# yukw777/EILEV

Measured on AMD Instinct MI355X. Metric: clips/sec (8-frame, 16 in-context) encode+generate, eilev-blip2-opt-2.7b, higher is better.
Workload: dtype bf16

## Files before the change

eilev_amd/csrc/common.h:

```cpp
#pragma once
#include <hip/hip_runtime.h>
#include <stdint.h>

#include <type_traits>

#include "../../include/eilev.h"

typedef __bf16 bf16;
typedef __attribute__((ext_vector_type(8))) __bf16 bf16x8;
typedef __attribute__((ext_vector_type(4))) __bf16 bf16x4;
typedef __attribute__((ext_vector_type(2))) __bf16 bf16x2;
typedef __attribute__((ext_vector_type(4))) float f32x4;
typedef __attribute__((ext_vector_type(16))) float f32x16;

#define EILEV_HIP_CHECK(expr)                          \
    do {                                               \
        hipError_t _e = (expr);                        \
        if (_e != hipSuccess) return (int)_e;          \
    } while (0)

static inline int eilev_num_cu() {
    static int n = 0;
    if (!n) {
        int dev = 0, cu = 0;
// ... 211 lines not shown
    DBG_GEMM_NB_BLOCKS_ONLY = 1 << 30,

    DBG_ATTN_NO_COMPUTE = 1 << 0,
    DBG_ATTN_NO_PREFETCH = 1 << 1,
    DBG_ATTN_NO_FRAME = 1 << 2,
    DBG_ATTN_FRAME3 = 1 << 4,
    DBG_ATTN_NO_FRAME3 = 1 << 5,
    DBG_ATTN_V2_4WAVES = 1 << 6,
    DBG_ATTN_FRAME_STAMPS = 1 << 8,
    DBG_ATTN_FRAME3_STAMPS = 1 << 9,
    DBG_ATTN_HEAD_MAJOR = 1 << 10,
    DBG_ATTN_FRAME3_NO_STORES = 1 << 11,
};
enum GemmForce : int { FORCE_NONE = 0, FORCE_PP4 = 9, FORCE_W6 = 12, FORCE_64x128 = 13, FORCE_128x128 = 14, FORCE_SPLIT_K = 15 };

struct GemmArgs {
    const bf16 *A;
    int64_t lda;
    const bf16 *W;
    int64_t ldw;
    const bf16 *Wp = nullptr;
    int a_frag = 0, c_frag = 0, ln_frag = 0;
    int hm_tok = 0, hm_heads = 0, hm_hd = 0;
    const bf16 *bias;
    const bf16 *resid;
    int64_t ldr;
    void *C;
    int64_t ldc;
    int M, N, K;
    int epi;
    int out_f32;
    float scale;
    int scale_cols;
    int patch_group;
    int dbg;
    float *scratch;
    size_t scratch_bytes;
    const float *wscale = nullptr;
    const uint8_t *W8 = nullptr;
    bf16 *w8_scratch = nullptr;
    const uint8_t *A8 = nullptr;
    const float *ascale = nullptr;
    const float *ln_rows = nullptr;
    const float *ln_csum = nullptr;
    float *stat_out = nullptr;
    int64_t stat_ld = 0;
// ... 3 lines not shown
    int k_slice = 0;
    unsigned long long *trace = nullptr;
    int trace_tiles = 0;
};

__host__ __device__ static inline int64_t frag32_index(int row, int col) { return (int64_t)(col >> 5) * 1024 + row * 32 + (col & 31); }

#ifdef EILEV_PROBES
extern int g_gemm_form;
#define GEMM_FORM(code) (g_gemm_form = (g_gemm_form & ~0xffff) | (code))
#define GEMM_FORM_BIT(bit) (g_gemm_form |= (bit))
extern int g_gemm_ks;
#define GEMM_FORM_KS(n) (g_gemm_ks = (n))
#else
#define GEMM_FORM(code) ((void)0)
#define GEMM_FORM_BIT(bit) ((void)0)
#define GEMM_FORM_KS(n) ((void)0)
#endif
enum : int { GEMM_FORM_ROW_CHUNKS = 1 << 16, GEMM_FORM_W8_EXPANDED = 1 << 17, GEMM_FORM_SPLIT_K = 1 << 18, GEMM_FORM_REDUCE_LN = 1 << 19,
             GEMM_FORM_STREAM_LAYOUT = 1 << 20 };

int launch_gemm(const GemmArgs &g, int prof_kind, hipStream_t s);
bool gemm_rows32_takes(const GemmArgs &g);
int launch_pp4_ext(const GemmArgs &g, int grid, hipStream_t s);
#ifdef EILEV_PROBES
#define EILEV_TRACE_M16 true
#else
#define EILEV_TRACE_M16 false
#endif
static inline bool pp4_all_lean(const GemmArgs &g) {
    const bool scale_ok = g.scale_cols == 0 || (g.scale_cols % 16 == 0 && g.epi == 0 && !g.resid && !g.ln_rows && !g.stat_out);
    return g.N % 128 == 0 && !g.out_f32 && g.patch_group == 0 && scale_ok && !g.wscale && !g.ascale && !g.dbg && (!g.trace || EILEV_TRACE_M16);
}
static inline bool hm_takes(const GemmArgs &g) {
    return g.hm_tok >= 128 && g.hm_heads > 0 && g.hm_hd > 64 && g.hm_hd % 8 == 0 && g.N == 3 * g.hm_heads * g.hm_hd && g.ln_rows && g.epi == 0 && !g.resid &&
           !g.stat_out && !g.scale_cols && pp4_all_lean(g) && g.N % 64 == 0 && g.M % g.hm_tok == 0 && (int64_t)g.M * g.N * 2 < 0xfffffff0ll;
}
bool gemv_rows_ok(int M, int N, int K);
int launch_gemv_rows(int pro, const bf16 *x, int64_t ldx, const bf16 *gamma, const bf16 *beta, float eps, const float *part, int heads, int hd,
                     int nsplit, const bf16 *W, const bf16 *bias, const bf16 *resid, int64_t ldr, void *out, int64_t ldo, int out_f32, int M, int N,
                     int K, int epi, float scale, int scale_cols, hipStream_t s);
bool gemv1_ok(int N, int K, int pro);
int launch_gemv1(int pro, const bf16 *x, const bf16 *gamma, const bf16 *beta, float eps, const bf16 *W, const bf16 *bias, const bf16 *resid, void *out,
                 int out_f32, int N, int K, int epi, float scale, int scale_cols, hipStream_t s, const float *part = nullptr, int heads = 0, int hd = 0,
                 int nsplit = 0);
bool gemvm_ok(int M, int N, int K, int pro);
// ... 111 lines not shown
```

eilev_amd/csrc/gemm.hip:

```cpp
#include "gemm_common.h"
#include "gemm_tiled.h"
#include "gemm_pp4.h"
#include "gemm_w6.h"
#include "gemm_skinny.h"

int g_eilev_grid_cus = 0;
#ifdef EILEV_PROBES
int g_gemm_debug = 0;
extern "C" int eilev_debug_gemm_flags(int f) { g_gemm_debug = f; return 0; }
extern "C" int eilev_debug_grid_cus(int n) { g_eilev_grid_cus = n; return 0; }
int g_gemm_form = 0;
int g_gemm_ks = 0;
#endif
#ifdef EILEV_PROBES
unsigned long long *g_gemm_trace = nullptr;
int g_gemm_trace_tiles = 0;
extern "C" int eilev_debug_gemm_trace(void *buf, int tiles) { g_gemm_trace = (unsigned long long *)buf; g_gemm_trace_tiles = tiles; return 0; }
#endif

namespace {

#ifndef EILEV_A3_MIN_K
#define EILEV_A3_MIN_K 5120
#endif
// ... 44 lines not shown
    if ((g.K % 128) || g.lda != g.K || g.ldw != g.K || ((uintptr_t)g.A8 & 15) || ((uintptr_t)g.W8 & 15) || g.patch_group != 0 ||
        (int64_t)g.M * g.K >= kOffsetLimit || (int64_t)g.N * g.K >= kOffsetLimit)
        return EILEV_E_UNSUPPORTED;
    if (!g.out_f32 && ((g.ldc & 7) || (g.N & 3) || ((uintptr_t)g.C & 15) || (g.resid && ((g.ldr & 7) || ((uintptr_t)g.resid & 15))))) return EILEV_E_UNSUPPORTED;
    return profiled(launch_pp4, g, prof_kind, s);
}

bool w8_streams(const GemmArgs &g) { return g.M <= 32 && g.K % 256 == 0 && g.patch_group == 0; }
int w8_check(const GemmArgs &g) {
    if (!g.A || !g.C || !g.wscale || g.N <= 0 || g.K <= 0 || g.ldw != g.K || ((uintptr_t)g.W8 & 15) || (g.K & 15)) return EILEV_E_BADARG;
    if (!w8_streams(g) && !g.w8_scratch) return EILEV_E_WORKSPACE;
    return EILEV_OK;
}
int w8_expand(const GemmArgs &g, hipStream_t s) {
    const int64_t n16 = (int64_t)g.N * g.K / 16;
    hipLaunchKernelGGL(w8_expand_kernel, dim3((unsigned)ceil_div64(n16, 256)), dim3(256), 0, s, g.W8, g.w8_scratch, n16);
    EILEV_LAUNCH_CHECK();
    return EILEV_OK;
}

bool ln_fold(const GemmArgs &g) { return g.ln_rows != nullptr || g.stat_out != nullptr; }
bool skinny_dma_ok(const GemmArgs &g) { return g.K % 256 == 0 && (!(g.dbg & DBG_GEMM_SKINNY_NO_DMA) || g.W8); }
bool skinny_takes(const GemmArgs &g) { return (g.M <= 16 || (g.M <= 32 && skinny_dma_ok(g))) && g.patch_group == 0 && !ln_fold(g); }

int check_args(const GemmArgs &g) {
    if (!g.A || !g.W || !g.C || g.N <= 0 || g.K <= 0) return EILEV_E_BADARG;
    if ((g.K & 7) || (g.lda & 7) || (g.ldw & 7) || ((uintptr_t)g.A & 15) || ((uintptr_t)g.W & 15)) return EILEV_E_UNSUPPORTED;
    if (g.hm_tok && (!hm_takes(g) || !fits_offset(g.M, g.lda))) return EILEV_E_UNSUPPORTED;
    if (ln_fold(g) && (g.W8 || g.wscale || g.out_f32 || g.patch_group || g.scale_cols || g.K % BK || !fits_offset(g.N, g.ldw))) return EILEV_E_UNSUPPORTED;
    const bool skinny = skinny_takes(g);
    if ((g.a_frag || g.c_frag || g.ln_frag) && !skinny) return EILEV_E_UNSUPPORTED;
    if (!skinny && !g.out_f32 && ((g.ldc & 7) || (g.N & 3) || ((uintptr_t)g.C & 15) || (g.resid && ((g.ldr & 7) || ((uintptr_t)g.resid & 15))) ||
                                   (g.bias && ((uintptr_t)g.bias & 7))))
        return EILEV_E_UNSUPPORTED;
    return EILEV_OK;
}


int skinny_nbsel(const GemmArgs &g, int nb, int ks) {
    int nbsel = (g.dbg >> DBG_GEMM_NB_SHIFT) & 7;
    if (nbsel == 0 && g.M > 16) {
        const int wgs = (g.dbg & DBG_GEMM_NB_BLOCKS_ONLY) ? nb : nb * ks;
        nbsel = wgs >= 8 * 240 ? 8 : (wgs >= 4 * 240 ? 4 : (wgs >= 2 * 240 ? 2 : 1));
    }
    if (nbsel == 7) nbsel = 8;
    if (nbsel != 2 && nbsel != 4 && nbsel != 8) nbsel = 1;
    if (nbsel == 8 && g.M <= 16) nbsel = 4;
    return g.W8 ? 1 : nbsel;
}

template <int MB, int NB>
int launch_skinny_nb(const SkinnyArgs &a, int nb, hipStream_t s) {
    const size_t sm = 4 * 2 * 8192 + (size_t)2 * 4 * MB * 64 * 4 * 4;
// ... 118 lines not shown
    return g.N % 256 == 0 ? 1.06 * fill(tiles256) < fill(tm256 * ceil_div64(g.N, 128)) : tiles256 < 1024;
}

bool split_k_takes(const GemmArgs &g) {
    return g.out_f32 && !g.bias && !g.resid && g.epi == 0 && !g.wscale && g.scale_cols == 0 && g.patch_group == 0 && g.K % BK == 0 && g.K >= 8192 &&
           ceil_div64(g.M, 128) * ceil_div64(g.N, 128) <= 128 && fits_offset(g.M, g.lda) && fits_offset(g.N, g.ldw);
}
int launch_split_k(const GemmArgs &g, hipStream_t s) {
    const int tiles = (int)(ceil_div64(g.M, 128) * ceil_div64(g.N, 128)), nk = g.K / BK;
    int slices = 512 / tiles;
    slices = slices < 2 ? 2 : (slices > 16 ? 16 : slices);
    if (slices > nk / 8) slices = nk / 8 > 1 ? nk / 8 : 1;
    GemmArgs gs = g;
    gs.k_slice = (nk + slices - 1) / slices;
    slices = (nk + gs.k_slice - 1) / gs.k_slice;
    if (g.ldc == g.N) EILEV_HIP_CHECK(hipMemsetAsync(g.C, 0, (size_t)g.M * g.N * sizeof(float), s));
    else EILEV_HIP_CHECK(hipMemset2DAsync(g.C, (size_t)g.ldc * sizeof(float), 0, (size_t)g.N * sizeof(float), (size_t)g.M, s));
    GEMM_FORM(3000 + slices);
    return eilev_launch<gemm_glds_kernel<128, 128, 2, 2, 0, 2, 2, 0>>(dim3(tiles, slices), dim3(256), 2 * (128 + 128) * 128, s, gs);
}

bool t64x128_takes(const GemmArgs &g) { return ceil_div64(g.M, 128) * ceil_div64(g.N, 128) < 96 && g.M > 64; }

int launch_wide(const GemmArgs &g, hipStream_t s) {
    const int force = (g.dbg >> DBG_GEMM_FORCE_SHIFT) & 15;
    const bool no_dma = g.dbg & DBG_GEMM_NO_DMA;
    int cfg = tile_cfg(g);
    bool promoted = false;
    if (cfg == CFG_256x128_1S && g.K % BK == 0 && !(g.dbg & DBG_GEMM_NO_WIDE)) cfg = CFG_256x256, promoted = true;
    if (cfg == CFG_256x128 && w6_ok(g) && force == FORCE_NONE && !(g.dbg & (DBG_GEMM_NO_WIDE | DBG_GEMM_NO_W6 | DBG_GEMM_NO_DMA))) cfg = CFG_256x256, promoted = true;
    if (force == FORCE_PP4) cfg = CFG_256x256;
    if (force == FORCE_64x128 || force == FORCE_128x128 || force == FORCE_SPLIT_K) cfg = CFG_128x128;
    else if (force >= CFG_256x256 && force <= CFG_128x128) cfg = force;

    if (w6_ok(g) && (force == FORCE_W6 || (force == FORCE_NONE && cfg == CFG_256x256 && w6_pick(g) && !(g.dbg & (DBG_GEMM_NO_W6 | DBG_GEMM_NO_DMA)))))
        return launch_w6(g, s);
    switch (cfg) {
        case CFG_256x256:
            if (!(promoted && (g.dbg & DBG_GEMM_WIDE_TILED)) && (force == FORCE_NONE || force == FORCE_PP4) && !no_dma && g.K % BK == 0 && fits_offset(g.N, g.ldw))
                return launch_pp4(g, s);
            return launch_tiled<256, 256, 2, 4, 2, 2>(g, s);
        case CFG_256x128_1S: return launch_tiled<256, 128, 4, 2, 1, 4, 1>(g, s);
        case CFG_256x128: return launch_tiled<256, 128, 4, 2, 2, 2>(g, s);
        default:
            if (split_k_takes(g) && (force == FORCE_NONE || force == FORCE_SPLIT_K) && !no_dma) return launch_split_k(g, s);
            if ((force == FORCE_64x128 || (force == FORCE_NONE && t64x128_takes(g))) && g.M > 64 && !no_dma) return launch_tiled<64, 128, 1, 2, 2, 3>(g, s);
            return launch_tiled<128, 128, 2, 2, 2, 2>(g, s);
    }
}

}


static int launch_gemm_core(const GemmArgs &g_in, int prof_kind, hipStream_t s, bool *ln_done);

bool gemm_rows32_takes(const GemmArgs &g) {
    if (!g.A || !g.W || !g.C || g.W8 || g.wscale || g.M <= 16 || g.M > 32 || g.K % 256 || g.patch_group || g.ln_rows || g.stat_out) return false;
    if ((g.lda & 7) || (g.ldw & 7) || ((uintptr_t)g.A & 15) || ((uintptr_t)g.W & 15) || (g.dbg & DBG_GEMM_NO_ROWS32)) return false;
    SkinnyArgs a;
    a.g = g;
    a.mr = 32;
    int ks = 1, ksteps = 0, grid_x = 0;
    return rows32_plan(g, (g.N + 15) / 16, skinny_n_cu(), a, ks, ksteps, grid_x);
}

extern "C" int eilev_stream_layout_pack(const void *w, int64_t n, int64_t k, void *out, void *stream) {
    if (!w || !out || w == out || n < 1 || k < 1) return EILEV_E_BADARG;
    if (n > 0x7fffffff || k > 0x7fffffff || n * k > 0x7fffffff0ll) return EILEV_E_UNSUPPORTED;
    int ks = 0, ksteps = 0, grid_x = 0;
    if (!rows32_shape((int)n, (int)k, skinny_n_cu(), ks, ksteps, grid_x)) return EILEV_E_UNSUPPORTED;
    const int64_t chunks = n * (k >> 3);
    hipLaunchKernelGGL(stream_pack_kernel, dim3((unsigned)((chunks + 255) / 256)), dim3(256), 0, (hipStream_t)stream, (const bf16 *)w, (bf16 *)out, (int)n, (int)k, grid_x);
    EILEV_LAUNCH_CHECK();
    return EILEV_OK;
}

int launch_gemm(const GemmArgs &g, int prof_kind, hipStream_t s) {
    bool ln_done = false;
    if (g.ln_out && g.M > 0 && (g.out_f32 || g.patch_group || (g.N & 7) || g.N > 4096 || (g.ldc & 7))) return EILEV_E_UNSUPPORTED;
    const int rc = launch_gemm_core(g, prof_kind, s, &ln_done);
    if (rc != EILEV_OK || !g.ln_out || ln_done || g.M <= 0) return rc;
    if (g.out_f32 || g.patch_group) return EILEV_E_UNSUPPORTED;
    if (!g.ln_beta) return launch_rmsnorm(reinterpret_cast<const bf16 *>(g.C), g.ldc, g.ln_gamma, g.ln_out, g.N, g.M, g.N, g.ln_eps, s);
    return launch_layernorm(reinterpret_cast<const bf16 *>(g.C), g.ldc, g.ln_gamma, g.ln_beta, g.ln_out, g.N, g.M, g.N, g.ln_eps, s);
}

static int launch_gemm_core(const GemmArgs &g_in, int prof_kind, hipStream_t s, bool *ln_done) {
    GemmArgs g = with_probes(g_in);
    if (g.M <= 0) return EILEV_OK;
    if (g.A8) return launch_a8w8(g, prof_kind, s);
    if (g.W8) {
        const int rc = w8_check(g);
        if (rc != EILEV_OK) return rc;
        if (!w8_streams(g)) {
            const int rc_x = w8_expand(g, s);
            if (rc_x != EILEV_OK) return rc_x;
            GEMM_FORM_BIT(GEMM_FORM_W8_EXPANDED);
            GemmArgs e = g_in;
            e.W = g.w8_scratch;
            e.W8 = nullptr;
            return launch_gemm_core(e, prof_kind, s, ln_done);
        }
        g.W = reinterpret_cast<const bf16 *>(g.W8);
    }
    const int rc = check_args(g);
    if (rc != EILEV_OK) return rc;
    if (skinny_takes(g)) return launch_skinny(g, s, ln_done);
    if (const int64_t rows = chunk_rows(g)) return launch_row_chunks(g_in, rows, prof_kind, s);
    return profiled(ln_fold(g) ? launch_pp4 : launch_wide, g, prof_kind, s);
}

#ifdef EILEV_PROBES
struct EilevDebugGemmArgs {
    const void *A; int64_t lda;
    const void *W; int64_t ldw;
    const void *bias, *resid; int64_t ldr;
    void *C; int64_t ldc;
    int32_t M, N, K, epi, out_f32;
    float scale;
    int32_t scale_cols, patch_group, hm_tok, hm_heads, hm_hd, pad0;
    const float *wscale;
    const void *W8;
    void *w8_scratch;
    const void *A8;
    const float *ascale, *ln_rows, *ln_csum;
    float *stat_out; int64_t stat_ld;
    const void *ln_gamma, *ln_beta;
    void *ln_out;
    float ln_eps;
    int32_t pad1;
// ... 42 lines not shown
```

eilev_amd/csrc/gemm_pp4.h:

```cpp
#pragma once
#include "gemm_common.h"

namespace {

#ifndef EILEV_PP4_DEEP
#define EILEV_PP4_DEEP 1
#endif
template <int EPI, bool F8 = false, int LN = 0, int M16K = 0, bool A3 = false>
__global__ __launch_bounds__(512, 2) void gemm_pp4_kernel(const GemmArgs g) {
    constexpr bool M16 = M16K != 0, HT16 = M16K == 2;
    constexpr bool TALL = HT16 && !A3;
    constexpr int TALL_BM = 384;
    constexpr int HT_WM = TALL ? TALL_BM / 4 : 64, HT_TM16 = HT_WM / 16;
    static_assert(!M16 || !F8, "16 x 16 form: bf16 instances");
    constexpr int BM = 256, BN = 256, NWM = 2, NWN = 4, NW = 8;
    constexpr int WM = BM / NWM, WN = BN / NWN, TM = WM / 32, TN = WN / 32;
    constexpr int STEP = (BM + BN) * 128;
    constexpr int PC = 8;
    static_assert(!A3 || M16, "A3: lean epilogues only");
    constexpr int STG0 = A3 ? 2 * BM * 128 : 2 * STEP;

    extern __shared__ __attribute__((aligned(16))) char smem[];
    auto a_slot = [&](int st) { return smem + (A3 ? (st % 3) * (BM * 128) : (st & 1) * STEP); };
    auto w_slot = [&](int st) { return smem + (A3 ? 3 * (BM * 128) + (st & 1) * (BN * 128) : (st & 1) * STEP + BM * 128); };
// ... 254 lines not shown
            if (hm) {
                const int TOK = g.hm_tok, HD = g.hm_hd, NH = g.hm_heads, D3 = g.N / 3;
                const int n0 = cn0 + coff;
                const int plane = __builtin_amdgcn_readfirstlane(n0 / D3), rr = n0 - plane * D3;
                int2 ent;
                if (rr < NH * 64) {
                    ent.x = (plane * NH + (rr >> 6)) * TOK * HD + schunk * 8;
                    ent.y = 64;
                } else {
                    const int cph = (HD - 64) >> 3, jb = ((rr - NH * 64) >> 3) + schunk, hh = jb / cph;
                    ent.x = (plane * NH + hh) * TOK * HD + TOK * 64 + (jb - hh * cph) * 8;
                    ent.y = HD - 64;
                }
                const int fw = __builtin_amdgcn_readfirstlane(r0 / TOK);
                const int m0 = r0 + srow, f0 = m0 / TOK;
                hm_t = m0 - f0 * TOK;
                hm_str2 = __builtin_amdgcn_readfirstlane(ent.y * 2);
                hm_off = (unsigned)(((f0 - fw) * TOK * g.N + ent.x + hm_t * ent.y) * 2);
                hm_off_w = hm_off + (unsigned)(TOK * g.N * 2) - (unsigned)(TOK * hm_str2);
                const int64_t left = ((int64_t)g.M / TOK - fw) * TOK * g.N * 2;
                rch = uniform_rsrc(reinterpret_cast<bf16 *>(g.C) + (int64_t)fw * TOK * g.N, (int)(unsigned)(left < 0xfffffff0ll ? left : 0xfffffff0ll));
            }
        }
        u32x4_t rv[4];
        auto res_load = [&](int u) {
#pragma unroll
            for (int it = 0; it < 4; ++it) rv[it] = __builtin_amdgcn_raw_buffer_load_b128(rr, rs_voff, (u * 32 + it * 8) * (int)(g.ldr * 2), 0);
        };
        if constexpr (RES) res_load(0);
        bf16x4 biasr[M16 ? 1 : TN][4];
        bf16x4 biasr16[M16 ? TN16 : 1];
        if constexpr (M16) {
#pragma unroll
            for (int j = 0; j < TN16; ++j) {
                if (g.bias) biasr16[j] = *reinterpret_cast<const bf16x4 *>(g.bias + cn0 + coff + j * 16 + g4 * 4);
                else biasr16[j] = (bf16x4){(bf16)0.f, (bf16)0.f, (bf16)0.f, (bf16)0.f};
            }
        } else {
#pragma unroll
        for (int j = 0; j < TN; ++j)
#pragma unroll
            for (int q = 0; q < 4; ++q) {
                if (g.bias) biasr[j][q] = *reinterpret_cast<const bf16x4 *>(g.bias + cn0 + wn * WN + j * 32 + q * 8 + hi * 4);
                else biasr[j][q] = (bf16x4){(bf16)0.f, (bf16)0.f, (bf16)0.f, (bf16)0.f};
            }
        }
// ... 116 lines not shown
                    if (g4 == 0) __builtin_amdgcn_raw_buffer_store_b64(__builtin_bit_cast(u32x2_t, t), rst, (U * 32 + ib * 16 + l15) * 8, 0, 0);
                }
            } else if constexpr (LNP) {
                typedef __attribute__((ext_vector_type(2))) unsigned u32x2_t;
                const f32x2_t t = (f32x2_t){st1 + __shfl_xor(st1, 32), st2 + __shfl_xor(st2, 32)};
                if (hi == 0) __builtin_amdgcn_raw_buffer_store_b64(__builtin_bit_cast(u32x2_t, t), rst, (U * 32 + l31) * 8, 0, 0);
            }
            __builtin_amdgcn_sched_barrier(0);
            bf16x8 erb[2];
#pragma unroll
            for (int h2 = 0; h2 < 2; ++h2) {
#pragma unroll
                for (int b = 0; b < 2; ++b) {
                    const int row = (h2 * 2 + b) * 8 + srow;
                    erb[b] = *reinterpret_cast<const bf16x8 *>(stg + row * 128 + ((schunk ^ (row & 7)) << 4));
                }
                if (hm) {
                    if constexpr (HMI) {
#pragma unroll
                        for (int b = 0; b < 2; ++b) {
                            const int RO = U * 32 + (h2 * 2 + b) * 8;
                            const unsigned vo = hm_t + RO >= g.hm_tok ? hm_off_w : hm_off;
                            __builtin_amdgcn_raw_buffer_store_b128(__builtin_bit_cast(u32x4_t, erb[b]), rch, vo, RO * hm_str2, EILEV_HM_AUX);
                        }
                    }
                } else {
#pragma unroll
                for (int b = 0; b < 2; ++b)
                    __builtin_amdgcn_raw_buffer_store_b128(__builtin_bit_cast(u32x4_t, erb[b]), rc, st_voff, (U * 32 + (h2 * 2 + b) * 8) * (int)(g.ldc * 2), EILEV_ST_AUX);
                }
            }
            asm volatile("s_nop 1" ::: "memory");
            __builtin_amdgcn_sched_barrier(0);
        });
    };
#define PP_WAIT_LGKM0() __builtin_amdgcn_s_waitcnt(0xC07F)
#define PP_WAIT_LGKM0_VM0() __builtin_amdgcn_s_waitcnt(0x0070)
#define PP_WAIT_VM0() __builtin_amdgcn_s_waitcnt(0x0F70)
#define PP_BARRIER()                       \
    do {                                   \
        __builtin_amdgcn_sched_barrier(0); \
        __builtin_amdgcn_s_barrier();      \
        __builtin_amdgcn_sched_barrier(0); \
    } while (0)

    int t = blockIdx.x, m0, n0;
// ... 256 lines not shown
```

eilev_amd/csrc/opt.hip:

```cpp
#include "stages.h"

namespace {
inline int64_t opt_ws_rows(int64_t M) { return (M > 16 && M < 32) ? 32 : M; }

}

OptBufs carve_opt(const EilevDims *d, int64_t M, void *ws) {
    Carver cv{(char *)ws};
    OptBufs b;
    M = opt_ws_rows(M);
    b.h = cv.take<bf16>((size_t)M * d->t_hidden);
    b.x = cv.take<bf16>((size_t)M * d->t_hidden);
    b.att = cv.take<bf16>((size_t)M * d->t_hidden);
    b.qkv = cv.take<bf16>((size_t)M * 3 * d->t_hidden);
    b.ffn = cv.take<bf16>((size_t)M * d->t_ffn);
    b.pid = cv.take<int32_t>((size_t)M);
    b.scratch = cv.take<float>(kSkinnyScratch / sizeof(float));
    b.a8 = cv.take<uint8_t>((size_t)M * (d->t_ffn > d->t_hidden ? d->t_ffn : d->t_hidden));
    b.a8_scale = cv.take<float>((size_t)M);
    b.used = cv.used;
    return b;
}

extern "C" size_t eilev_opt_workspace_bytes(const EilevDims *d, int64_t batch, int64_t seq_len) {
// ... 9 lines not shown
    if (!w8 || !sc) return EILEV_E_BADARG;
    if (w->w8_act_fp8 && g.M > 32 && g.K % 128 == 0 && (int64_t)g.M * g.K < 0x7fff0000ll && (int64_t)g.N * g.K < 0x7fff0000ll) {
        RC(launch_quant_rows_e4m3(g.A, g.lda, b.a8, b.a8_scale, g.M, g.K, s));
        g.A8 = b.a8;
        g.ascale = b.a8_scale;
        g.lda = g.K;
        g.W8 = w8;
        g.wscale = sc;
        g.ldw = g.K;
        return EILEV_OK;
    }
    if (g.M > 32 || g.K % 256 != 0) {
        if (!w->w8_expand || w->w8_expand_bytes < (size_t)g.N * g.K * sizeof(bf16)) return EILEV_E_WORKSPACE;
        g.w8_scratch = (bf16 *)w->w8_expand;
    }
    g.W8 = w8;
    g.wscale = sc;
    g.ldw = g.K;
    return EILEV_OK;
}

}

int opt_qkv(const EilevDims *d, const EilevOptWeights *w, int l, const OptBufs &b, int64_t M, hipStream_t s, int a_frag) {
    const EilevOptLayer *L = &w->layers[l];
    const int D = d->t_hidden;
    const float scaling = 1.0f / sqrtf((float)(D / d->t_heads));
    const void *ws[3] = {L->q_w, L->k_w, L->v_w}, *bs[3] = {L->q_b, L->k_b, L->v_b};
    const bool bias_fused = packed(bs, 3, D);
    if (w->layers_w8) {
        if (!bias_fused && (L->q_b || L->k_b || L->v_b)) return EILEV_E_UNSUPPORTED;
        GemmArgs g = sk_gemm(b.scratch, b.x, D, nullptr, D, L->q_b, nullptr, 0, b.qkv, 3 * D, M, 3 * D, D, 0);
        g.scale = scaling; g.scale_cols = D;
        RC(use_w8(g, w, w->layers_w8[l].qkv_w8, w->layers_w8[l].qkv_scale, b, s));
        return launch_gemm(g, 5, s);
    }
    const bool fused = packed(ws, 3, (size_t)D * D) && bias_fused;
    for (int i = 0; i < (fused ? 1 : 3); ++i) {
        GemmArgs g = sk_gemm(b.scratch, b.x, D, ws[i], D, bs[i], nullptr, 0, b.qkv + i * D, 3 * D, M, fused ? 3 * D : D, D, 0);
        if (i == 0) { g.scale = scaling; g.scale_cols = D; }
        if (fused && w->layers_stream && M > 16 && M <= 32) g.Wp = (const bf16 *)w->layers_stream[l].qkv_s;
        g.a_frag = a_frag;
        RC(launch_gemm(g, 5, s));
    }
    return EILEV_OK;
}

int opt_tail(const EilevDims *d, const EilevOptWeights *w, int l, const OptBufs &b, int64_t M, hipStream_t s, const void *next_ln_w,
             const void *next_ln_b, int frag, bool dry) {
    const EilevOptLayer *L = &w->layers[l];
    const EilevOptLayerW8 *Q = w->layers_w8 ? &w->layers_w8[l] : nullptr;
    const int D = d->t_hidden, Ft = d->t_ffn;
    const EilevOptLayerStream *S = (w->layers_stream && !Q && M > 16 && M <= 32) ? &w->layers_stream[l] : nullptr;
    GemmArgs g = sk_gemm(b.scratch, b.att, D, L->o_w, D, L->o_b, b.h, D, b.h, D, M, D, D, 0);
    g.ln_gamma = (const bf16 *)L->ln2_w; g.ln_beta = (const bf16 *)L->ln2_b; g.ln_out = b.x; g.ln_eps = d->t_eps;
    if (S) g.Wp = (const bf16 *)S->o_s;
    g.a_frag = g.ln_frag = frag;
    if (dry && !gemm_rows32_takes(g)) return EILEV_E_UNSUPPORTED;
    if (Q) RC(use_w8(g, w, Q->o_w8, Q->o_scale, b, s));
    if (!dry) RC(launch_gemm(g, 5, s));
    g = sk_gemm(b.scratch, b.x, D, L->fc1_w, D, L->fc1_b, nullptr, 0, b.ffn, Ft, M, Ft, D, 2);
    if (S) g.Wp = (const bf16 *)S->fc1_s;
    g.a_frag = g.c_frag = frag;
    if (dry && !gemm_rows32_takes(g)) return EILEV_E_UNSUPPORTED;
    if (Q) RC(use_w8(g, w, Q->fc1_w8, Q->fc1_scale, b, s));
    if (!dry) RC(launch_gemm(g, 5, s));
    g = sk_gemm(b.scratch, b.ffn, Ft, L->fc2_w, Ft, L->fc2_b, b.h, D, b.h, D, M, D, Ft, 0);
    if (S) g.Wp = (const bf16 *)S->fc2_s;
    if (next_ln_w) {
        g.ln_gamma = (const bf16 *)next_ln_w; g.ln_beta = (const bf16 *)next_ln_b; g.ln_out = b.x; g.ln_eps = d->t_eps;
    }
    g.a_frag = frag;
    g.ln_frag = next_ln_w ? frag : 0;
    if (dry) return gemm_rows32_takes(g) ? EILEV_OK : EILEV_E_UNSUPPORTED;
    if (Q) RC(use_w8(g, w, Q->fc2_w8, Q->fc2_scale, b, s));
    return launch_gemm(g, 5, s);
}

namespace {
int g_decode_frag = 1;
}
int g_decode_rows = 1;
#ifdef EILEV_PROBES
extern "C" int eilev_debug_decode_rows(int on) { g_decode_rows = on; return 0; }
extern "C" int eilev_debug_decode_frag(int on) { g_decode_frag = on; return 0; }
#endif
namespace {

bool opt_qkv_packed(const EilevDims *d, const EilevOptWeights *w) {
    const int D = d->t_hidden;
    for (int l = 0; l < d->t_layers; ++l) {
        const EilevOptLayer *L = &w->layers[l];
        const void *ws[3] = {L->q_w, L->k_w, L->v_w}, *bs[3] = {L->q_b, L->k_b, L->v_b};
        if (!packed(ws, 3, (size_t)D * D) || !L->q_b || !packed(bs, 3, D)) return false;
    }
    return true;
}
bool opt_rows_usable(const EilevDims *d, const EilevOptWeights *w, int64_t M) {
    if (!g_decode_rows || w->layers_w8 || M > 2) return false;
    const int D = d->t_hidden;
    return gemv_rows_ok((int)M, D, D) && gemv_rows_ok((int)M, D, d->t_ffn) && (D / d->t_heads) % 8 == 0 && opt_qkv_packed(d, w);
}
bool opt_rows1_usable(const EilevDims *d, const EilevOptWeights *w, int64_t M, int64_t cap) {
    if (M != 1 || g_decode_rows == 3 || !opt_rows_usable(d, w, M)) return false;
    const int D = d->t_hidden;
    return gemv1_ok(3 * D, D, 1) && gemv1_ok(D, D, 0) && gemv1_ok(d->t_ffn, D, 1) && gemv1_ok(D, d->t_ffn, 0) && gemv1_ok(d->vocab, D, 1) &&
           attn_decode1_ok(1, (int)cap, D / d->t_heads);
}
// ... 75 lines not shown
            int nsplit = 0;
            RC(opt_rows_qkv(d, w, l, b, M, s));
            RC(launch_attn_decode(al, s, &nsplit));
            RC(opt_rows_tail(d, w, l, b, M, al.part, nsplit, s));
        }
        return opt_rows_head(d, w, b, M, logits, s);
    }
    const int D = d->t_hidden;
    for (int l = 0; l < d->t_layers; ++l) {
        const EilevOptLayer *L = &w->layers[l];
        DecodeAttnArgs al = at_block(a, l, kv_layer, gen_layer);
        al.out_frag = frag;
        if (l == 0) RC(launch_layernorm(b.h, D, (const bf16 *)L->ln1_w, (const bf16 *)L->ln1_b, b.x, D, M, D, d->t_eps, s));
        RC(opt_qkv(d, w, l, b, M, s, l > 0 ? frag : 0));
        RC(launch_attn_decode(al, s));
        const bool last = l + 1 == d->t_layers;
        RC(opt_tail(d, w, l, b, M, s, last ? w->final_ln_w : w->layers[l + 1].ln1_w, last ? w->final_ln_b : w->layers[l + 1].ln1_b, frag));
    }
    GemmArgs g = opt_lm_head(d, w, b, M, logits);
    g.a_frag = frag;
    return launch_gemm(g, 5, s);
}

int opt_blocks(const EilevDims *d, const EilevOptWeights *w, const OptBufs &b, const void *inputs_embeds, const int32_t *attn_mask, int64_t batch,
               int64_t rows, int64_t past_len, bool from_cache, void *kv_cache, int64_t kv_capacity, void *hidden, hipStream_t s) {
    const int D = d->t_hidden, H = d->t_heads, hd = D / H;
    const int64_t M = batch * rows, total = past_len + rows;
    RC(launch_pos_embed((const bf16 *)inputs_embeds, (const bf16 *)w->embed_positions, attn_mask, b.pid, b.h, (int)batch, (int)total, D,
                        s, (int)past_len));
    const KvCache kv(batch, D, kv_capacity);
    const size_t hs_bytes = (size_t)M * D * sizeof(bf16);
    for (int l = 0; l < d->t_layers; ++l) {
        const EilevOptLayer *L = &w->layers[l];
        bf16 *kc = kv.k((bf16 *)kv_cache, l), *vc = kv.v((bf16 *)kv_cache, l);
        if (hidden) RC(copy_hidden(hidden, l, b.h, hs_bytes, s));
        RC(launch_layernorm(b.h, D, (const bf16 *)L->ln1_w, (const bf16 *)L->ln1_b, b.x, D, M, D, d->t_eps, s));
        RC(opt_qkv(d, w, l, b, M, s));
        RC(launch_kv_write(b.qkv, kc, vc, (int)batch, (int)rows, H, hd, (int)kv_capacity, (int)total, nullptr, s, (int)past_len));
        AttnArgs a = from_cache ? attn_cache(b.qkv, 3 * D, kc, vc, kv_capacity, b.att, batch, H, rows, total, hd, 1.0f)
                                : attn_rows(b.qkv, 3 * D, b.qkv + D, 3 * D, b.qkv + 2 * D, 3 * D, b.att, batch, H, rows, total, hd, 1.0f);
        a.causal = 1; a.key_mask = attn_mask; a.mask_ld = total;
        RC(launch_attention(a, s));
        RC(opt_tail(d, w, l, b, M, s));
    }
    RC(launch_layernorm(b.h, D, (const bf16 *)w->final_ln_w, (const bf16 *)w->final_ln_b, b.x, D, M, D, d->t_eps, s));
    if (hidden) RC(copy_hidden(hidden, d->t_layers, b.x, hs_bytes, s));
    return EILEV_OK;
}

int opt_prefill_impl(const EilevDims *d, const EilevOptWeights *w, const void *inputs_embeds, const int32_t *attn_mask, int64_t batch,
                     int64_t seq_len, void *kv_cache, int64_t kv_capacity, float *logits_last, float *logits_all, void *hidden,
                     void *workspace, size_t workspace_bytes, void *stream) {
    if (!d || !w || !inputs_embeds || !attn_mask || !kv_cache || !workspace || batch <= 0 || seq_len <= 0) return EILEV_E_BADARG;
    if (seq_len > kv_capacity || seq_len > d->max_pos) return EILEV_E_BADARG;
    if (!dims_ok_opt(d)) return EILEV_E_UNSUPPORTED;
    if (workspace_bytes < eilev_opt_workspace_bytes(d, batch, seq_len)) return EILEV_E_WORKSPACE;
    hipStream_t s = (hipStream_t)stream;
    const int D = d->t_hidden;
    const int64_t M = batch * seq_len;
    const OptBufs b = carve_opt(d, M, workspace);
    RC(opt_blocks(d, w, b, inputs_embeds, attn_mask, batch, seq_len, 0, false, kv_cache, kv_capacity, hidden, s));
    if (logits_all) {
        GemmArgs g = mk_gemm(b.x, D, w->embed_tokens, D, nullptr, nullptr, 0, logits_all, d->vocab, M, d->vocab, D, 0);
        g.out_f32 = 1;
        RC(launch_gemm(g, 5, s));
    }
    if (logits_last) {
        GemmArgs g = sk_gemm(b.scratch, b.x + (seq_len - 1) * (int64_t)D, seq_len * (int64_t)D, w->embed_tokens, D, nullptr, nullptr, 0,
                             logits_last, d->vocab, batch, d->vocab, D, 0);
        g.out_f32 = 1;
        RC(launch_gemm(g, 5, s));
    }
    return EILEV_OK;
}
}

extern "C" int eilev_opt_prefill(const EilevDims *d, const EilevOptWeights *w, const void *inputs_embeds,
                                 const int32_t *attn_mask, int64_t batch, int64_t seq_len, void *kv_cache, int64_t kv_capacity,
                                 float *logits_last, float *logits_all, void *workspace, size_t workspace_bytes, void *stream) {
    return opt_prefill_impl(d, w, inputs_embeds, attn_mask, batch, seq_len, kv_cache, kv_capacity, logits_last, logits_all, nullptr, workspace,
                            workspace_bytes, stream);
}
extern "C" int eilev_opt_prefill_debug(const EilevDims *d, const EilevOptWeights *w, const void *inputs_embeds,
                                       const int32_t *attn_mask, int64_t batch, int64_t seq_len, void *kv_cache, int64_t kv_capacity,
                                       float *logits_last, float *logits_all, void *hidden_states, void *workspace, size_t workspace_bytes,
                                       void *stream) {
    if (!hidden_states) return EILEV_E_BADARG;
    return opt_prefill_impl(d, w, inputs_embeds, attn_mask, batch, seq_len, kv_cache, kv_capacity, logits_last, logits_all, hidden_states,
                            workspace, workspace_bytes, stream);
}

extern "C" int eilev_opt_extend(const EilevDims *d, const EilevOptWeights *w, const void *inputs_embeds, const int32_t *attn_mask,
                                int64_t batch, int64_t new_len, int64_t past_len, void *kv_cache, int64_t kv_capacity,
                                float *logits_all, void *workspace, size_t workspace_bytes, void *stream) {
    if (!d || !w || !inputs_embeds || !attn_mask || !kv_cache || !logits_all || !workspace || batch <= 0 || new_len <= 0 || past_len < 0)
        return EILEV_E_BADARG;
    const int64_t total = past_len + new_len;
    if (total > kv_capacity || total > d->max_pos) return EILEV_E_BADARG;
    if (!dims_ok_opt(d)) return EILEV_E_UNSUPPORTED;
    if (workspace_bytes < eilev_opt_workspace_bytes(d, batch, total)) return EILEV_E_WORKSPACE;
    hipStream_t s = (hipStream_t)stream;
    const int D = d->t_hidden;
    const int64_t M = batch * new_len;
    const OptBufs b = carve_opt(d, batch * total, workspace);
    RC(opt_blocks(d, w, b, inputs_embeds, attn_mask, batch, new_len, past_len, true, kv_cache, kv_capacity, nullptr, s));
    GemmArgs g = sk_gemm(b.scratch, b.x, D, w->embed_tokens, D, nullptr, nullptr, 0, logits_all, d->vocab, M, d->vocab, D, 0);
    g.out_f32 = 1;
    return launch_gemm(g, 5, s);
}

extern "C" int eilev_greedy_select(const float *logits, int64_t batch, int64_t vocab, int32_t *state, uint8_t *finished,
                                   int64_t eos_id, int64_t pad_id, int64_t *tokens, int64_t *out_tokens, int64_t max_new,
                                   void *stream) {
    if (!logits || !state || !finished || !tokens || !out_tokens || batch <= 0) return EILEV_E_BADARG;
    return launch_select(logits, (int)batch, (int)vocab, state, finished, eos_id, pad_id, tokens, out_tokens, max_new,
                         (hipStream_t)stream);
}

extern "C" int eilev_topk_logprob(const float *logits, const float *row_score, int64_t rows, int64_t vocab, int64_t keep, float *out_val,
                                  int32_t *out_idx, void *stream) {
    if (!logits || !out_val || !out_idx || rows < 0 || vocab <= 0 || keep <= 0 || keep > vocab) return EILEV_E_BADARG;
    if (rows == 0) return EILEV_OK;
    return launch_topk_logprob(logits, row_score, (int)rows, (int)vocab, (int)keep, out_val, out_idx, (hipStream_t)stream);
}

extern "C" size_t eilev_beam_scratch_bytes(int64_t batch, int64_t beams, int64_t keep, int64_t max_new) {
    return sizeof(int64_t) * (size_t)batch * (size_t)(keep + 2 * beams) * (size_t)max_new;
}
// ... 125 lines not shown
```

eilev_amd/csrc/stages.h:

```cpp
#pragma once
#include "common.h"

#define RC(expr)                 \
    do {                         \
        int _rc = (expr);        \
        if (_rc != 0) return _rc; \
    } while (0)

struct Carver {
    char *base;
    size_t used = 0;
    template <typename T>
    T *take(size_t n) {
        T *q = base ? reinterpret_cast<T *>(base + used) : nullptr;
        used += align_up(n * sizeof(T), 256);
        return q;
    }
};

static inline GemmArgs mk_gemm(const bf16 *A, int64_t lda, const void *W, int64_t ldw, const void *bias, const bf16 *resid, int64_t ldr,
                               void *C, int64_t ldc, int64_t M, int N, int K, int epi) {
    GemmArgs g;
    g.A = A; g.lda = lda; g.W = (const bf16 *)W; g.ldw = ldw; g.bias = (const bf16 *)bias; g.resid = resid; g.ldr = ldr;
    g.C = C; g.ldc = ldc; g.M = (int)M; g.N = N; g.K = K; g.epi = epi; g.out_f32 = 0; g.scale = 1.0f; g.scale_cols = 0;
// ... 57 lines not shown
}

struct T5BeamArgs {
    int64_t beams;
    const void *kv_start;
    void *kv_gen;
    int64_t gen_capacity;
    const int32_t *ancestors;
};
int t5_decode_step_beam(const EilevT5Dims *d, const EilevT5Weights *w, const int64_t *tokens, int32_t *state, const int32_t *enc_mask,
                        int64_t rows, const T5BeamArgs &beam, const void *cross_kv, int64_t enc_len, float *logits, void *workspace,
                        size_t workspace_bytes, void *stream);
size_t t5_decode_step_beam_workspace_bytes(const EilevT5Dims *d, int64_t rows, int64_t enc_len, int64_t gen_capacity);

struct OptBufs {
    bf16 *h, *x, *att, *qkv, *ffn;
    int32_t *pid;
    float *scratch;
    uint8_t *a8;
    float *a8_scale;
    size_t used;
};
OptBufs carve_opt(const EilevDims *d, int64_t M, void *ws);
int opt_qkv(const EilevDims *d, const EilevOptWeights *w, int l, const OptBufs &b, int64_t M, hipStream_t s, int a_frag = 0);
int opt_tail(const EilevDims *d, const EilevOptWeights *w, int l, const OptBufs &b, int64_t M, hipStream_t s, const void *next_ln_w = nullptr,
             const void *next_ln_b = nullptr, int frag = 0, bool dry = false);

int opt_decode_step_beam(const EilevDims *d, const EilevOptWeights *w, const int64_t *tokens, int32_t *state, const int32_t *attn_mask,
                         const int32_t *n_valid, int64_t rows, int64_t beams, int64_t seq_len, const void *kv_prompt, void *kv_gen, int64_t gen_capacity,
                         const int32_t *ancestors, float *logits, void *workspace, size_t workspace_bytes, void *stream, int shared_prompt);
size_t opt_decode_step_beam_shared_bytes(const EilevDims *d, int64_t rows, int64_t seq_len, int64_t gen_capacity);

extern int g_decode_rows;
```

Baseline: 231.5.

## Write prefill K/V directly from QKV GEMM and compute only last rows in final layer

The fused QKV GEMM epilogue in the pp4 kernel can now store K and V columns straight into the KV cache layout, which removes the separate kv_write kernel during prompt prefill. Attention then reads K/V from the cache. In the last OPT layer, the output projection, FFN and final layernorm run only on each sequence's last row, because only last-token logits are needed. Tile routing keeps the full-M shape so the smaller GEMMs still pick the same kernels. This adds epilogue complexity and a routing override, and relies on the last-rows path being used only when the full hidden states and all-position logits are not requested.

```diff
diff --git a/eilev_amd/csrc/common.h b/eilev_amd/csrc/common.h
--- a/eilev_amd/csrc/common.h
+++ b/eilev_amd/csrc/common.h
@@ -257,6 +257,9 @@
     const bf16 *Wp = nullptr;
     int a_frag = 0, c_frag = 0, ln_frag = 0;
     int hm_tok = 0, hm_heads = 0, hm_hd = 0;
+    bf16 *kv_k = nullptr, *kv_v = nullptr;
+    int kv_seq = 0, kv_cap = 0, kv_heads = 0, kv_hd = 0;
+    int route_m = 0;
     const bf16 *bias;
     const bf16 *resid;
     int64_t ldr;
@@ -306,6 +309,7 @@
 
 int launch_gemm(const GemmArgs &g, int prof_kind, hipStream_t s);
 bool gemm_rows32_takes(const GemmArgs &g);
+bool gemm_kv_takes(const GemmArgs &g);
 int launch_pp4_ext(const GemmArgs &g, int grid, hipStream_t s);
 #ifdef EILEV_PROBES
 #define EILEV_TRACE_M16 true
diff --git a/eilev_amd/csrc/gemm.hip b/eilev_amd/csrc/gemm.hip
--- a/eilev_amd/csrc/gemm.hip
+++ b/eilev_amd/csrc/gemm.hip
@@ -90,13 +90,23 @@
 bool ln_fold(const GemmArgs &g) { return g.ln_rows != nullptr || g.stat_out != nullptr; }
 bool skinny_dma_ok(const GemmArgs &g) { return g.K % 256 == 0 && (!(g.dbg & DBG_GEMM_SKINNY_NO_DMA) || g.W8); }
 bool skinny_takes(const GemmArgs &g) { return (g.M <= 16 || (g.M <= 32 && skinny_dma_ok(g))) && g.patch_group == 0 && !ln_fold(g); }
+GemmArgs route_shape(const GemmArgs &g) {
+    GemmArgs r = g;
+    if (g.route_m > 0) r.M = g.route_m;
+    return r;
+}
+bool route_ok(const GemmArgs &g) {
+    return g.route_m == 0 || (g.route_m > 32 && g.M <= g.route_m && !g.out_f32 && !g.patch_group && !ln_fold(g) && !g.W8 && !g.A8 && !g.wscale &&
+                              !g.hm_tok && !g.kv_k && !g.a_frag && !g.c_frag && !g.ln_frag && fits_offset(g.M, g.lda));
+}
 
 int check_args(const GemmArgs &g) {
     if (!g.A || !g.W || !g.C || g.N <= 0 || g.K <= 0) return EILEV_E_BADARG;
     if ((g.K & 7) || (g.lda & 7) || (g.ldw & 7) || ((uintptr_t)g.A & 15) || ((uintptr_t)g.W & 15)) return EILEV_E_UNSUPPORTED;
     if (g.hm_tok && (!hm_takes(g) || !fits_offset(g.M, g.lda))) return EILEV_E_UNSUPPORTED;
+    if (!route_ok(g)) return EILEV_E_UNSUPPORTED;
     if (ln_fold(g) && (g.W8 || g.wscale || g.out_f32 || g.patch_group || g.scale_cols || g.K % BK || !fits_offset(g.N, g.ldw))) return EILEV_E_UNSUPPORTED;
-    const bool skinny = skinny_takes(g);
+    const bool skinny = skinny_takes(route_shape(g));
     if ((g.a_frag || g.c_frag || g.ln_frag) && !skinny) return EILEV_E_UNSUPPORTED;
     if (!skinny && !g.out_f32 && ((g.ldc & 7) || (g.N & 3) || ((uintptr_t)g.C & 15) || (g.resid && ((g.ldr & 7) || ((uintptr_t)g.resid & 15))) ||
                                    (g.bias && ((uintptr_t)g.bias & 7))))
@@ -261,10 +271,12 @@
 
 bool t64x128_takes(const GemmArgs &g) { return ceil_div64(g.M, 128) * ceil_div64(g.N, 128) < 96 && g.M > 64; }
 
-int launch_wide(const GemmArgs &g, hipStream_t s) {
+enum WideRoute : int { WIDE_W6, WIDE_PP4, WIDE_256x256, WIDE_256x128_1S, WIDE_256x128, WIDE_SPLIT_K, WIDE_64x128, WIDE_128x128 };
+WideRoute wide_route(const GemmArgs &g) {
+    const GemmArgs r = route_shape(g);
     const int force = (g.dbg >> DBG_GEMM_FORCE_SHIFT) & 15;
     const bool no_dma = g.dbg & DBG_GEMM_NO_DMA;
-    int cfg = tile_cfg(g);
+    int cfg = tile_cfg(r);
     bool promoted = false;
     if (cfg == CFG_256x128_1S && g.K % BK == 0 && !(g.dbg & DBG_GEMM_NO_WIDE)) cfg = CFG_256x256, promoted = true;
     if (cfg == CFG_256x128 && w6_ok(g) && force == FORCE_NONE && !(g.dbg & (DBG_GEMM_NO_WIDE | DBG_GEMM_NO_W6 | DBG_GEMM_NO_DMA))) cfg = CFG_256x256, promoted = true;
@@ -272,20 +284,43 @@
     if (force == FORCE_64x128 || force == FORCE_128x128 || force == FORCE_SPLIT_K) cfg = CFG_128x128;
     else if (force >= CFG_256x256 && force <= CFG_128x128) cfg = force;
 
-    if (w6_ok(g) && (force == FORCE_W6 || (force == FORCE_NONE && cfg == CFG_256x256 && w6_pick(g) && !(g.dbg & (DBG_GEMM_NO_W6 | DBG_GEMM_NO_DMA)))))
-        return launch_w6(g, s);
+    if (w6_ok(g) && (force == FORCE_W6 || (force == FORCE_NONE && cfg == CFG_256x256 && w6_pick(r) && !(g.dbg & (DBG_GEMM_NO_W6 | DBG_GEMM_NO_DMA)))))
+        return WIDE_W6;
     switch (cfg) {
         case CFG_256x256:
             if (!(promoted && (g.dbg & DBG_GEMM_WIDE_TILED)) && (force == FORCE_NONE || force == FORCE_PP4) && !no_dma && g.K % BK == 0 && fits_offset(g.N, g.ldw))
-                return launch_pp4(g, s);
-            return launch_tiled<256, 256, 2, 4, 2, 2>(g, s);
-        case CFG_256x128_1S: return launch_tiled<256, 128, 4, 2, 1, 4, 1>(g, s);
-        case CFG_256x128: return launch_tiled<256, 128, 4, 2, 2, 2>(g, s);
+                return WIDE_PP4;
+            return WIDE_256x256;
+        case CFG_256x128_1S: return WIDE_256x128_1S;
+        case CFG_256x128: return WIDE_256x128;
         default:
-            if (split_k_takes(g) && (force == FORCE_NONE || force == FORCE_SPLIT_K) && !no_dma) return launch_split_k(g, s);
-            if ((force == FORCE_64x128 || (force == FORCE_NONE && t64x128_takes(g))) && g.M > 64 && !no_dma) return launch_tiled<64, 128, 1, 2, 2, 3>(g, s);
-            return launch_tiled<128, 128, 2, 2, 2, 2>(g, s);
-    }
+            if (split_k_takes(g) && (force == FORCE_NONE || force == FORCE_SPLIT_K) && !no_dma) return WIDE_SPLIT_K;
+            if ((force == FORCE_64x128 || (force == FORCE_NONE && t64x128_takes(r))) && r.M > 64 && !no_dma) return WIDE_64x128;
+            return WIDE_128x128;
+    }
+}
+int launch_wide(const GemmArgs &g, hipStream_t s) {
+    switch (wide_route(g)) {
+        case WIDE_W6: return launch_w6(g, s);
+        case WIDE_PP4: return launch_pp4(g, s);
+        case WIDE_256x256: return launch_tiled<256, 256, 2, 4, 2, 2>(g, s);
+        case WIDE_256x128_1S: return launch_tiled<256, 128, 4, 2, 1, 4, 1>(g, s);
+        case WIDE_256x128: return launch_tiled<256, 128, 4, 2, 2, 2>(g, s);
+        case WIDE_SPLIT_K: return launch_split_k(g, s);
+        case WIDE_64x128: return launch_tiled<64, 128, 1, 2, 2, 3>(g, s);
+        default: return launch_tiled<128, 128, 2, 2, 2, 2>(g, s);
+    }
+}
+
+bool kv_shape_ok(const GemmArgs &g) {
+    const int64_t D = g.N / 3, plane2 = (int64_t)g.kv_heads * g.kv_cap * g.kv_hd * 2;
+    return g.kv_k && g.kv_v && g.kv_seq >= 128 && g.kv_cap >= g.kv_seq && g.kv_heads > 0 && g.kv_hd > 0 && g.kv_hd % 8 == 0 && g.N % 3 == 0 &&
+           D == (int64_t)g.kv_heads * g.kv_hd && D % 64 == 0 && g.N % 256 == 0 && g.M % g.kv_seq == 0 && ((uintptr_t)g.kv_k & 15) == 0 &&
+           ((uintptr_t)g.kv_v & 15) == 0 && ((int64_t)g.M / g.kv_seq + 4) * plane2 < kOffsetLimit;
+}
+bool kv_takes(const GemmArgs &g) {
+    return kv_shape_ok(g) && !g.A8 && !g.W8 && !g.wscale && !ln_fold(g) && !g.hm_tok && !g.route_m && !g.resid && g.epi == 0 && !g.out_f32 &&
+           !skinny_takes(g) && !chunk_rows(g) && pp4_all_lean(g) && !a3_takes(g) && wide_route(g) == WIDE_PP4;
 }
 
 }
@@ -303,6 +338,11 @@
     return rows32_plan(g, (g.N + 15) / 16, skinny_n_cu(), a, ks, ksteps, grid_x);
 }
 
+bool gemm_kv_takes(const GemmArgs &g_in) {
+    const GemmArgs g = with_probes(g_in);
+    return g.M > 0 && check_args(g) == EILEV_OK && kv_takes(g);
+}
+
 extern "C" int eilev_stream_layout_pack(const void *w, int64_t n, int64_t k, void *out, void *stream) {
     if (!w || !out || w == out || n < 1 || k < 1) return EILEV_E_BADARG;
     if (n > 0x7fffffff || k > 0x7fffffff || n * k > 0x7fffffff0ll) return EILEV_E_UNSUPPORTED;
@@ -327,6 +367,7 @@
 static int launch_gemm_core(const GemmArgs &g_in, int prof_kind, hipStream_t s, bool *ln_done) {
     GemmArgs g = with_probes(g_in);
     if (g.M <= 0) return EILEV_OK;
+    if ((g.route_m || g.kv_k) && (g.A8 || g.W8)) return EILEV_E_UNSUPPORTED;
     if (g.A8) return launch_a8w8(g, prof_kind, s);
     if (g.W8) {
         const int rc = w8_check(g);
@@ -344,7 +385,8 @@
     }
     const int rc = check_args(g);
     if (rc != EILEV_OK) return rc;
-    if (skinny_takes(g)) return launch_skinny(g, s, ln_done);
+    if (g.kv_k && !kv_takes(g)) return EILEV_E_UNSUPPORTED;
+    if (skinny_takes(route_shape(g))) return launch_skinny(g, s, ln_done);
     if (const int64_t rows = chunk_rows(g)) return launch_row_chunks(g_in, rows, prof_kind, s);
     return profiled(ln_fold(g) ? launch_pp4 : launch_wide, g, prof_kind, s);
 }
diff --git a/eilev_amd/csrc/gemm_pp4.h b/eilev_amd/csrc/gemm_pp4.h
--- a/eilev_amd/csrc/gemm_pp4.h
+++ b/eilev_amd/csrc/gemm_pp4.h
@@ -300,6 +300,26 @@
                 rch = uniform_rsrc(reinterpret_cast<bf16 *>(g.C) + (int64_t)fw * TOK * g.N, (int)(unsigned)(left < 0xfffffff0ll ? left : 0xfffffff0ll));
             }
         }
+        constexpr bool KVI = LN == 0 && !RES && EPI == 0 && M16K == 2 && !A3 && !HTE && !F8;
+        bool kv = false;
+        unsigned kv_off = 0, kv_off_w = 0;
+        int kv_pos = 0, kv_str2 = 0;
+        if constexpr (KVI) {
+            const int n0 = cn0 + coff, D = g.N / 3;
+            if (g.kv_k != nullptr && n0 >= D) {
+                kv = true;
+                const int which = __builtin_amdgcn_readfirstlane(n0 >= 2 * D ? 1 : 0);
+                const int c = n0 - (1 + which) * D + schunk * 8;
+                const int head = c / g.kv_hd, dim = c - head * g.kv_hd;
+                const int m0 = r0 + srow, b0 = m0 / g.kv_seq;
+                const int sample = g.kv_heads * g.kv_cap * g.kv_hd;
+                kv_pos = m0 - b0 * g.kv_seq;
+                kv_str2 = __builtin_amdgcn_readfirstlane(g.kv_hd * 2);
+                kv_off = (unsigned)((b0 * sample + (head * g.kv_cap + kv_pos) * g.kv_hd + dim) * 2);
+                kv_off_w = kv_off + (unsigned)((sample - g.kv_seq * g.kv_hd) * 2);
+                rch = uniform_rsrc(which ? g.kv_v : g.kv_k, (g.M / g.kv_seq) * sample * 2);
+            }
+        }
         u32x4_t rv[4];
         auto res_load = [&](int u) {
 #pragma unroll
@@ -462,6 +482,15 @@
                             const int RO = U * 32 + (h2 * 2 + b) * 8;
                             const unsigned vo = hm_t + RO >= g.hm_tok ? hm_off_w : hm_off;
                             __builtin_amdgcn_raw_buffer_store_b128(__builtin_bit_cast(u32x4_t, erb[b]), rch, vo, RO * hm_str2, EILEV_HM_AUX);
+                        }
+                    }
+                } else if (kv) {
+                    if constexpr (KVI) {
+#pragma unroll
+                        for (int b = 0; b < 2; ++b) {
+                            const int RO = U * 32 + (h2 * 2 + b) * 8;
+                            const unsigned vo = (kv_pos + RO >= g.kv_seq ? kv_off_w : kv_off) + (unsigned)(RO * kv_str2);
+                            __builtin_amdgcn_raw_buffer_store_b128(__builtin_bit_cast(u32x4_t, erb[b]), rch, vo, 0, EILEV_ST_AUX);
                         }
                     }
                 } else {
diff --git a/eilev_amd/csrc/opt.hip b/eilev_amd/csrc/opt.hip
--- a/eilev_amd/csrc/opt.hip
+++ b/eilev_amd/csrc/opt.hip
@@ -55,7 +55,7 @@
 
 }
 
-int opt_qkv(const EilevDims *d, const EilevOptWeights *w, int l, const OptBufs &b, int64_t M, hipStream_t s, int a_frag) {
+int opt_qkv(const EilevDims *d, const EilevOptWeights *w, int l, const OptBufs &b, int64_t M, hipStream_t s, int a_frag, OptKvDest *kv) {
     const EilevOptLayer *L = &w->layers[l];
     const int D = d->t_hidden;
     const float scaling = 1.0f / sqrtf((float)(D / d->t_heads));
@@ -74,6 +74,11 @@
         if (i == 0) { g.scale = scaling; g.scale_cols = D; }
         if (fused && w->layers_stream && M > 16 && M <= 32) g.Wp = (const bf16 *)w->layers_stream[l].qkv_s;
         g.a_frag = a_frag;
+        if (kv && fused) {
+            GemmArgs gk = g;
+            gk.kv_k = kv->k; gk.kv_v = kv->v; gk.kv_seq = (int)kv->seq; gk.kv_cap = (int)kv->cap; gk.kv_heads = d->t_heads; gk.kv_hd = D / d->t_heads;
+            if (kv->seq <= 0x7fffffff && kv->cap <= 0x7fffffff && gemm_kv_takes(gk)) g = gk, kv->done = true;
+        }
         RC(launch_gemm(g, 5, s));
     }
     return EILEV_OK;
@@ -111,12 +116,16 @@
 }
 
 namespace {
+int g_prefill_passes = 1;
+int g_prefill_took = 0;
 int g_decode_frag = 1;
 }
 int g_decode_rows = 1;
 #ifdef EILEV_PROBES
 extern "C" int eilev_debug_decode_rows(int on) { g_decode_rows = on; return 0; }
 extern "C" int eilev_debug_decode_frag(int on) { g_decode_frag = on; return 0; }
+extern "C" int eilev_debug_prefill_passes(int on) { g_prefill_passes = on; return 0; }
+extern "C" int eilev_debug_prefill_took() { const int t = g_prefill_took; g_prefill_took = 0; return t; }
 #endif
 namespace {
 
@@ -238,8 +247,31 @@
     return launch_gemm(g, 5, s);
 }
 
+bf16 *opt_last_x(const OptBufs &b, int64_t batch, int D) { return b.qkv + batch * D; }
+bool opt_last_rows_usable(const EilevDims *d, const EilevOptWeights *w, int64_t batch, int64_t seq_len) {
+    const int64_t M = batch * seq_len;
+    return g_prefill_passes && !w->layers_w8 && seq_len > 1 && M > 32 && M * (int64_t)d->t_ffn * 2 < 0x7fff0000ll;
+}
+int opt_tail_last_rows(const EilevDims *d, const EilevOptWeights *w, int l, const OptBufs &b, int64_t batch, int64_t seq_len, hipStream_t s) {
+    const EilevOptLayer *L = &w->layers[l];
+    const int D = d->t_hidden, Ft = d->t_ffn;
+    const int64_t M = batch * seq_len, last = (seq_len - 1) * (int64_t)D, ld = seq_len * (int64_t)D;
+    bf16 *hc = b.qkv;
+    GemmArgs g = sk_gemm(b.scratch, b.att + last, ld, L->o_w, D, L->o_b, b.h + last, ld, hc, D, batch, D, D, 0);
+    g.ln_gamma = (const bf16 *)L->ln2_w; g.ln_beta = (const bf16 *)L->ln2_b; g.ln_out = b.x; g.ln_eps = d->t_eps;
+    g.route_m = (int)M;
+    RC(launch_gemm(g, 5, s));
+    g = sk_gemm(b.scratch, b.x, D, L->fc1_w, D, L->fc1_b, nullptr, 0, b.ffn, Ft, batch, Ft, D, 2);
+    g.route_m = (int)M;
+    RC(launch_gemm(g, 5, s));
+    g = sk_gemm(b.scratch, b.ffn, Ft, L->fc2_w, Ft, L->fc2_b, hc, D, hc, D, batch, D, Ft, 0);
+    g.route_m = (int)M;
+    RC(launch_gemm(g, 5, s));
+    return launch_layernorm(hc, D, (const bf16 *)w->final_ln_w, (const bf16 *)w->final_ln_b, opt_last_x(b, batch, D), D, batch, D, d->t_eps, s);
+}
+
 int opt_blocks(const EilevDims *d, const EilevOptWeights *w, const OptBufs &b, const void *inputs_embeds, const int32_t *attn_mask, int64_t batch,
-               int64_t rows, int64_t past_len, bool from_cache, void *kv_cache, int64_t kv_capacity, void *hidden, hipStream_t s) {
+               int64_t rows, int64_t past_len, bool from_cache, void *kv_cache, int64_t kv_capacity, void *hidden, bool last_rows, hipStream_t s) {
     const int D = d->t_hidden, H = d->t_heads, hd = D / H;
     const int64_t M = batch * rows, total = past_len + rows;
     RC(launch_pos_embed((const bf16 *)inputs_embeds, (const bf16 *)w->embed_positions, attn_mask, b.pid, b.h, (int)batch, (int)total, D,
@@ -251,12 +283,16 @@
         bf16 *kc = kv.k((bf16 *)kv_cache, l), *vc = kv.v((bf16 *)kv_cache, l);
         if (hidden) RC(copy_hidden(hidden, l, b.h, hs_bytes, s));
         RC(launch_layernorm(b.h, D, (const bf16 *)L->ln1_w, (const bf16 *)L->ln1_b, b.x, D, M, D, d->t_eps, s));
-        RC(opt_qkv(d, w, l, b, M, s));
-        RC(launch_kv_write(b.qkv, kc, vc, (int)batch, (int)rows, H, hd, (int)kv_capacity, (int)total, nullptr, s, (int)past_len));
-        AttnArgs a = from_cache ? attn_cache(b.qkv, 3 * D, kc, vc, kv_capacity, b.att, batch, H, rows, total, hd, 1.0f)
+        OptKvDest kvd = {kc, vc, rows, kv_capacity, false};
+        const bool kv_direct = g_prefill_passes && past_len == 0 && !from_cache && !hidden;
+        RC(opt_qkv(d, w, l, b, M, s, 0, kv_direct ? &kvd : nullptr));
+        if (kvd.done) g_prefill_took |= 1;
+        if (!kvd.done) RC(launch_kv_write(b.qkv, kc, vc, (int)batch, (int)rows, H, hd, (int)kv_capacity, (int)total, nullptr, s, (int)past_len));
+        AttnArgs a = from_cache || kvd.done ? attn_cache(b.qkv, 3 * D, kc, vc, kv_capacity, b.att, batch, H, rows, total, hd, 1.0f)
                                 : attn_rows(b.qkv, 3 * D, b.qkv + D, 3 * D, b.qkv + 2 * D, 3 * D, b.att, batch, H, rows, total, hd, 1.0f);
         a.causal = 1; a.key_mask = attn_mask; a.mask_ld = total;
         RC(launch_attention(a, s));
+        if (last_rows && l + 1 == d->t_layers) return g_prefill_took |= 2, opt_tail_last_rows(d, w, l, b, batch, rows, s);
         RC(opt_tail(d, w, l, b, M, s));
     }
     RC(launch_layernorm(b.h, D, (const bf16 *)w->final_ln_w, (const bf16 *)w->final_ln_b, b.x, D, M, D, d->t_eps, s));
@@ -275,14 +311,15 @@
     const int D = d->t_hidden;
     const int64_t M = batch * seq_len;
     const OptBufs b = carve_opt(d, M, workspace);
-    RC(opt_blocks(d, w, b, inputs_embeds, attn_mask, batch, seq_len, 0, false, kv_cache, kv_capacity, hidden, s));
+    const bool last_rows = !logits_all && !hidden && opt_last_rows_usable(d, w, batch, seq_len);
+    RC(opt_blocks(d, w, b, inputs_embeds, attn_mask, batch, seq_len, 0, false, kv_cache, kv_capacity, hidden, last_rows, s));
     if (logits_all) {
         GemmArgs g = mk_gemm(b.x, D, w->embed_tokens, D, nullptr, nullptr, 0, logits_all, d->vocab, M, d->vocab, D, 0);
         g.out_f32 = 1;
         RC(launch_gemm(g, 5, s));
     }
     if (logits_last) {
-        GemmArgs g = sk_gemm(b.scratch, b.x + (seq_len - 1) * (int64_t)D, seq_len * (int64_t)D, w->embed_tokens, D, nullptr, nullptr, 0,
+        GemmArgs g = sk_gemm(b.scratch, last_rows ? opt_last_x(b, batch, D) : b.x + (seq_len - 1) * (int64_t)D, last_rows ? D : seq_len * (int64_t)D, w->embed_tokens, D, nullptr, nullptr, 0,
                              logits_last, d->vocab, batch, d->vocab, D, 0);
         g.out_f32 = 1;
         RC(launch_gemm(g, 5, s));
@@ -319,7 +356,7 @@
     const int D = d->t_hidden;
     const int64_t M = batch * new_len;
     const OptBufs b = carve_opt(d, batch * total, workspace);
-    RC(opt_blocks(d, w, b, inputs_embeds, attn_mask, batch, new_len, past_len, true, kv_cache, kv_capacity, nullptr, s));
+    RC(opt_blocks(d, w, b, inputs_embeds, attn_mask, batch, new_len, past_len, true, kv_cache, kv_capacity, nullptr, false, s));
     GemmArgs g = sk_gemm(b.scratch, b.x, D, w->embed_tokens, D, nullptr, nullptr, 0, logits_all, d->vocab, M, d->vocab, D, 0);
     g.out_f32 = 1;
     return launch_gemm(g, 5, s);
diff --git a/eilev_amd/csrc/stages.h b/eilev_amd/csrc/stages.h
--- a/eilev_amd/csrc/stages.h
+++ b/eilev_amd/csrc/stages.h
@@ -103,7 +103,12 @@
     size_t used;
 };
 OptBufs carve_opt(const EilevDims *d, int64_t M, void *ws);
-int opt_qkv(const EilevDims *d, const EilevOptWeights *w, int l, const OptBufs &b, int64_t M, hipStream_t s, int a_frag = 0);
+struct OptKvDest {
+    bf16 *k, *v;
+    int64_t seq, cap;
+    bool done;
+};
+int opt_qkv(const EilevDims *d, const EilevOptWeights *w, int l, const OptBufs &b, int64_t M, hipStream_t s, int a_frag = 0, OptKvDest *kv = nullptr);
 int opt_tail(const EilevDims *d, const EilevOptWeights *w, int l, const OptBufs &b, int64_t M, hipStream_t s, const void *next_ln_w = nullptr,
              const void *next_ln_b = nullptr, int frag = 0, bool dry = false);
 
```

Result: no change. 232.1, median of 6 (+0.3%).
